# tjhladish/AbcSmc

Measured on AMD Instinct MI355X. Metric: particles/sec per SMC generation (PLS+weight+resample), 1/2/4/8 GPU, higher is better.
Workload: dtype f64 (inputs, model, distances, proposals, results; pair sums of the weight stage: fp64 operands as three f16 limbs on the matrix pipe + f32 v_exp_f32, weights <= 5e-7 rel of the fp64 oracle, largest seen 3.1e-7); 1 GPU; configs[2]: synthetic 1M particles x 16 params x 32 metrics, PLS 8 components, full generation; particles_per_gpu=1000000, particles_total=1000000, metrics=32, params=16, pls_components=8, pred_prior_size=100000, prev_pred_prior_size=100000, next_set_size=1000000, noise=MULTIVARIATE, ncomp_chosen=8, pls_component_rule=wilcoxon, parallelism=row-sharded x1, launcher=single GPU

## Files before the change

abcsmc_amd/csrc/select.hip:

```cpp
#include "abc_internal.h"

namespace {

struct SelState {
    unsigned long long prefix;
    unsigned long long mask;
    unsigned long long krem;
    unsigned long long n_less;
    unsigned long long ties;
};

__device__ __forceinline__ unsigned long long key_of(double d) {
    const unsigned long long b = (unsigned long long)__double_as_longlong(d);
    return (b >> 63) ? ~b : (b | 0x8000000000000000ull);
}
__device__ __forceinline__ double dist_of(unsigned long long k) {
    const unsigned long long b = (k >> 63) ? (k & 0x7fffffffffffffffull) : ~k;
    return __longlong_as_double((long long)b);
}

constexpr int SEL_BITS = 11;
constexpr int SEL_BINS = 1 << SEL_BITS;

__global__ void k_sel_init(SelState* st, unsigned long long K, unsigned int* hist) {
    for (int i = threadIdx.x; i < SEL_BINS; i += blockDim.x) hist[i] = 0;
    if (threadIdx.x == 0) { st->prefix = 0; st->mask = 0; st->krem = K; st->n_less = 0; st->ties = 0; }
}

__global__ __launch_bounds__(256) void k_sel_hist(const double* __restrict__ dist, size_t n,
                                                  const SelState* __restrict__ st, int shift, int nbits,
                                                  unsigned int* __restrict__ hist) {
    __shared__ unsigned int lh[SEL_BINS];
    for (int i = threadIdx.x; i < SEL_BINS; i += 256) lh[i] = 0;
    __syncthreads();
    const unsigned long long prefix = st->prefix, mask = st->mask;
    const unsigned int dm = (1u << nbits) - 1u;
    const size_t stride = (size_t)gridDim.x * 256;
    const int lane = threadIdx.x & 63;
    const unsigned long long lt_mask = (lane == 0) ? 0ull : (~0ull >> (64 - lane));
    const size_t nround = (n + stride - 1) / stride;
    for (size_t it = 0; it < nround; it++) {
        const size_t i = it * stride + (size_t)blockIdx.x * 256 + threadIdx.x;
        const unsigned long long k = (i < n) ? key_of(dist[i]) : 0ull;
        const bool in = (i < n) && ((k & mask) == prefix);
        const unsigned int d = (unsigned int)(k >> shift) & dm;
        unsigned long long peers = __ballot(in);
        for (int b = 0; b < nbits; b++) {
            const unsigned long long m = __ballot((d >> b) & 1u);
            peers &= ((d >> b) & 1u) ? m : ~m;
        }
        if (in && (peers & lt_mask) == 0) atomicAdd(&lh[d], (unsigned int)__popcll(peers));
    }
    __syncthreads();
    for (int i = threadIdx.x; i < SEL_BINS; i += 256) {
        const unsigned int c = lh[i];
        if (c) atomicAdd(&hist[i], c);
    }
}

__device__ __forceinline__ SelState sel_pick_block(const unsigned int* __restrict__ hist, SelState st, int shift, int nbits,
                                                   int last, unsigned long long K, unsigned long long* csum ,
                                                   int* found_digit, unsigned long long* found_below) {
    const int t = threadIdx.x;
    const int bins = 1 << nbits;
    const int per = (bins + 255) / 256;
    unsigned long long loc = 0;
    for (int j = 0; j < per; j++) { const int b = t * per + j; if (b < bins) loc += hist[b]; }
    const int lane = t & 63, wave = t >> 6;
    unsigned long long inc = loc;
#pragma unroll
    for (int o = 1; o < 64; o <<= 1) {
        const unsigned long long up = __shfl_up(inc, o, 64);
        if (lane >= o) inc += up;
    }
    if (lane == 63) csum[wave] = inc;
    __syncthreads();
    unsigned long long run = inc - loc;
    for (int w = 0; w < wave; w++) run += csum[w];
    const unsigned long long krem = st.krem;
    for (int j = 0; j < per; j++) {
        const int b = t * per + j;
        if (b < bins) {
            const unsigned long long c = hist[b];
            if (run < krem && krem <= run + c) { *found_digit = b; *found_below = run; }
            run += c;
        }
    }
    __syncthreads();
    const unsigned long long dm = ((1ull << nbits) - 1ull) << shift;
    st.prefix |= ((unsigned long long)*found_digit) << shift;
    st.mask |= dm;
    st.krem = krem - *found_below;
    if (last) { st.ties = st.krem; st.n_less = K - st.krem; }
    __syncthreads();
    return st;
}

__global__ __launch_bounds__(256) void k_sel_pick(SelState* st, int shift, int nbits, unsigned int* hist,
                                                  int last, unsigned long long K) {
    __shared__ unsigned long long csum[256];
    __shared__ int found_digit;
    __shared__ unsigned long long found_below;
    const SelState nst = sel_pick_block(hist, *st, shift, nbits, last, K, csum, &found_digit, &found_below);
    if (threadIdx.x == 0) *st = nst;
    for (int i = threadIdx.x; i < SEL_BINS; i += 256) hist[i] = 0;
}

__global__ void k_sel_init_fused(SelState* st_arr , unsigned long long K, unsigned int* hist_all ) {
    for (int i = threadIdx.x; i < 6 * SEL_BINS; i += blockDim.x) hist_all[i] = 0;
    if (threadIdx.x == 0) { st_arr[0].prefix = 0; st_arr[0].mask = 0; st_arr[0].krem = K; st_arr[0].n_less = 0; st_arr[0].ties = 0; }
}

__global__ __launch_bounds__(256) void k_sel_hist_fused(const double* __restrict__ dist, size_t n, SelState* __restrict__ st_arr,
                                                        int p, int shift_prev, int nbits_prev, int shift, int nbits,
                                                        unsigned int* __restrict__ hist_all, unsigned long long K) {
    __shared__ unsigned int lh[SEL_BINS];
    __shared__ unsigned long long csum[256];
    __shared__ int found_digit;
    __shared__ unsigned long long found_below;
    SelState st = st_arr[p > 0 ? p - 1 : 0];
    if (p > 0) {
        st = sel_pick_block(hist_all + (size_t)(p - 1) * SEL_BINS, st, shift_prev, nbits_prev, 0, K, csum, &found_digit, &found_below);
        if (threadIdx.x == 0) st_arr[p] = st;
    }
    for (int i = threadIdx.x; i < SEL_BINS; i += 256) lh[i] = 0;
    __syncthreads();
    unsigned int* hist = hist_all + (size_t)p * SEL_BINS;
    const unsigned long long prefix = st.prefix, mask = st.mask;
    const unsigned int dm = (1u << nbits) - 1u;
    const size_t stride = (size_t)gridDim.x * 256;
    const int lane = threadIdx.x & 63;
    const unsigned long long lt_mask = (lane == 0) ? 0ull : (~0ull >> (64 - lane));
    const size_t nround = (n + stride - 1) / stride;
    for (size_t it = 0; it < nround; it++) {
        const size_t i = it * stride + (size_t)blockIdx.x * 256 + threadIdx.x;
        const unsigned long long k = (i < n) ? key_of(dist[i]) : 0ull;
        const bool in = (i < n) && ((k & mask) == prefix);
        const unsigned int d = (unsigned int)(k >> shift) & dm;
        unsigned long long peers = __ballot(in);
        for (int b = 0; b < nbits; b++) {
            const unsigned long long m = __ballot((d >> b) & 1u);
            peers &= ((d >> b) & 1u) ? m : ~m;
        }
        if (in && (peers & lt_mask) == 0) atomicAdd(&lh[d], (unsigned int)__popcll(peers));
    }
    __syncthreads();
    for (int i = threadIdx.x; i < SEL_BINS; i += 256) {
        const unsigned int c = lh[i];
        if (c) atomicAdd(&hist[i], c);
    }
}


constexpr int BS_NB = 4096;
constexpr int BS_NB_BIG = 16384;
constexpr int BS_S = 4096;
constexpr int BS_CAP = 1024;
constexpr int BS_CSTRIDE = 32;
struct BinSel {
    unsigned long long lo, hi;
    int shift;
    int bstar;
    unsigned long long need;
    int fail;
    int pad_;
};

__global__ __launch_bounds__(1024) void k_bs_sample(const double* __restrict__ dist, size_t n, unsigned long long K,
                                                    BinSel* __restrict__ bs, unsigned int* __restrict__ hist ,
                                                    int* __restrict__ fail_flag, int nbins) {
    __shared__ unsigned long long sk[BS_S];
    __shared__ unsigned int h[256];
    __shared__ unsigned long long red[16];
    __shared__ unsigned long long s_prefix;
    __shared__ unsigned int s_rank;
    const int t = threadIdx.x;
    for (int i = t; i < nbins + 1; i += 1024) hist[i] = 0;
    const size_t stride = n / BS_S;
    unsigned long long mn = ~0ull;
    {
        static_assert(BS_S % 1024 == 0 && BS_S / 1024 <= 8, "samples per thread");
        double dv[BS_S / 1024];
#pragma unroll
        for (int j = 0; j < BS_S / 1024; j++) dv[j] = dist[(size_t)(t + 1024 * j) * stride + stride / 2];
#pragma unroll
        for (int j = 0; j < BS_S / 1024; j++) {
            const unsigned long long k = key_of(dv[j]);
            sk[t + 1024 * j] = k;
            mn = k < mn ? k : mn;
        }
    }
#pragma unroll
    for (int o = 32; o >= 1; o >>= 1) { const unsigned long long v = __shfl_xor(mn, o, 64); mn = v < mn ? v : mn; }
    if ((t & 63) == 0) red[t >> 6] = mn;
    const double f = (double)K / (double)n;
    double qd = f * BS_S + 4.0 * sqrt(BS_S * f * (1.0 - f)) + 8.0;
    unsigned int q = (qd >= (double)(BS_S - 1)) ? BS_S - 1 : (unsigned int)qd;
    if (t == 0) { s_prefix = 0; s_rank = q; }
    __syncthreads();
    for (int w = 0; w < 16; w++) mn = red[w] < mn ? red[w] : mn;
    unsigned long long mask = 0;
    for (int pass = 0; pass < 3; pass++) {
        const int shift = 56 - 8 * pass;
        if (t < 256) h[t] = 0;
        __syncthreads();
        const unsigned long long prefix = s_prefix;
        for (int i = t; i < BS_S; i += 1024)
            if ((sk[i] & mask) == prefix) atomicAdd(&h[(unsigned int)(sk[i] >> shift) & 255u], 1u);
        __syncthreads();
        if (t < 64) {
            unsigned int c[4], sum = 0;
#pragma unroll
            for (int j = 0; j < 4; j++) { c[j] = h[4 * t + j]; sum += c[j]; }
            unsigned int inc = sum;
#pragma unroll
            for (int o = 1; o < 64; o <<= 1) { const unsigned int u = __shfl_up(inc, o, 64); if (t >= o) inc += u; }
            unsigned int run = inc - sum;
            const unsigned int r = s_rank;
#pragma unroll
            for (int j = 0; j < 4; j++) {
                if (run <= r && r < run + c[j]) { s_prefix = prefix | ((unsigned long long)(4 * t + j) << shift); s_rank = r - run; }
                run += c[j];
            }
        }
        mask |= 255ull << shift;
        __syncthreads();
    }
    if (t == 0) {
        const unsigned long long lo = mn, hi = s_prefix | ~mask;
        const unsigned long long span = hi - lo;
        int shift = 0;
        while (shift < 63 && (span >> shift) >= (unsigned long long)(nbins - 1)) shift++;
        bs->lo = lo; bs->hi = hi; bs->shift = shift; bs->bstar = 0; bs->need = 0; bs->fail = 0; bs->pad_ = 0;
        *fail_flag = 0;
    }
}

__device__ __forceinline__ int bs_bin(unsigned long long k, unsigned long long lo, int shift) {
    return (k <= lo) ? 0 : (int)((k - lo) >> shift);
}

__global__ __launch_bounds__(256) void k_bs_hist(const double* __restrict__ dist, size_t n, const BinSel* __restrict__ bs,
                                                 unsigned int* __restrict__ hist, unsigned int* __restrict__ cursor, int nbins) {
    extern __shared__ unsigned int lh[];
    for (size_t i = (size_t)blockIdx.x * 256 + threadIdx.x; i < (size_t)nbins * BS_CSTRIDE; i += (size_t)gridDim.x * 256) cursor[i] = 0;
    for (int i = threadIdx.x; i < nbins; i += 256) lh[i] = 0;
    __syncthreads();
    const unsigned long long lo = bs->lo, hi = bs->hi;
    const int shift = bs->shift;
    const size_t stride = (size_t)gridDim.x * 256;
    for (size_t i0 = (size_t)blockIdx.x * 256 + threadIdx.x; i0 < n; i0 += 8 * stride) {
        double d[8];
#pragma unroll
        for (int u = 0; u < 8; u++) { const size_t i = i0 + u * stride; d[u] = dist[i < n ? i : i0]; }
#pragma unroll
        for (int u = 0; u < 8; u++) {
            const unsigned long long k = key_of(d[u]);
            if (i0 + u * stride < n && k <= hi) atomicAdd(&lh[bs_bin(k, lo, shift)], 1u);
        }
    }
    __syncthreads();
    for (int i = threadIdx.x; i < nbins; i += 256) {
        const unsigned int c = lh[i];
        if (c) atomicAdd(&hist[i], c);
    }
}

template <int BPT>
__global__ __launch_bounds__(1024) void k_bs_scan(BinSel* __restrict__ bs, unsigned int* __restrict__ hist, unsigned long long K,
                                                  int* __restrict__ fail_flag) {
    __shared__ unsigned int wsum[16];
    __shared__ int s_fail;
    const int t = threadIdx.x, lane = t & 63, wave = t >> 6;
    if (t == 0) s_fail = 0;
    unsigned int c[BPT], sum = 0;
#pragma unroll
    for (int j = 0; j < BPT; j++) { c[j] = hist[BPT * t + j]; sum += c[j]; }
    unsigned int inc = sum;
#pragma unroll
    for (int o = 1; o < 64; o <<= 1) { const unsigned int u = __shfl_up(inc, o, 64); if (lane >= o) inc += u; }
    if (lane == 63) wsum[wave] = inc;
    __syncthreads();
    unsigned int run = inc - sum;
    for (int w = 0; w < wave; w++) run += wsum[w];
    unsigned int tot = 0;
    for (int w = 0; w < 16; w++) tot += wsum[w];
#pragma unroll
    for (int j = 0; j < BPT; j++) {
        const unsigned int off = run;
        hist[BPT * t + j] = off;
        if ((unsigned long long)off < K && K <= (unsigned long long)off + c[j]) { bs->bstar = BPT * t + j; bs->need = K - off; }
        if ((unsigned long long)off < K && c[j] > (unsigned int)BS_CAP) s_fail = 1;
        run += c[j];
    }
    if (t == 0) hist[BPT * 1024] = tot;
    __syncthreads();
    if (t == 0) {
        const int fail = (s_fail || (unsigned long long)tot < K) ? 1 : 0;
        bs->fail = fail;
        *fail_flag = fail;
    }
}

__global__ __launch_bounds__(256) void k_bs_scatter(const double* __restrict__ dist, size_t n, const BinSel* __restrict__ bs,
                                                    const unsigned int* __restrict__ offs, unsigned int* __restrict__ cursor,
                                                    unsigned long long idx_base, unsigned long long* __restrict__ tkey,
                                                    unsigned long long* __restrict__ tidx) {
    if (bs->fail) return;
    const unsigned long long lo = bs->lo, hi = bs->hi;
    const int shift = bs->shift, bstar = bs->bstar;
    const size_t i = (size_t)blockIdx.x * 256 + threadIdx.x;
    if (i >= n) return;
    const unsigned long long k = key_of(dist[i]);
    if (k > hi) return;
    const int b = bs_bin(k, lo, shift);
    if (b > bstar) return;
    const unsigned int p = offs[b] + atomicAdd(&cursor[(size_t)b * BS_CSTRIDE], 1u);
    tkey[p] = k;
    tidx[p] = idx_base + i;
}

__global__ __launch_bounds__(256) void k_bs_sort(const BinSel* __restrict__ bs, const unsigned int* __restrict__ offs,
                                                 const unsigned long long* __restrict__ tkey,
                                                 const unsigned long long* __restrict__ tidx, unsigned long long K,
                                                 unsigned long long idx_base, unsigned long long* __restrict__ oidx,
                                                 double* __restrict__ odist) {
    __shared__ unsigned long long sk[BS_CAP];
    __shared__ unsigned long long si[BS_CAP];
    const int b = blockIdx.x, t = threadIdx.x;
    if (bs->fail) {
        for (unsigned long long i = (unsigned long long)b * 256 + t; i < K; i += (unsigned long long)gridDim.x * 256) {
            oidx[i] = idx_base + i;
            if (odist) odist[i] = 0.0;
        }
        return;
    }
    if (b > bs->bstar) return;
    const unsigned int o0 = offs[b], cnt = offs[b + 1] - o0;
    if (cnt == 0) return;
    const unsigned int keep = (b == bs->bstar) ? (unsigned int)bs->need : cnt;
    unsigned int n2 = 2;
    while (n2 < cnt) n2 <<= 1;
    for (unsigned int e = t; e < n2; e += 256) {
        sk[e] = (e < cnt) ? tkey[o0 + e] : ~0ull;
        si[e] = (e < cnt) ? tidx[o0 + e] : ~0ull;
    }
    __syncthreads();
    for (unsigned int k = 2; k <= n2; k <<= 1)
        for (unsigned int j = k >> 1; j > 0; j >>= 1) {
            for (unsigned int p = t; p < n2 / 2; p += 256) {
                const unsigned int i = ((p & ~(j - 1)) << 1) | (p & (j - 1));
                const unsigned long long ka = sk[i], kb = sk[i + j], ia = si[i], ib = si[i + j];
                const bool gt = (ka > kb) || (ka == kb && ia > ib);
                if (gt == ((i & k) == 0)) { sk[i] = kb; sk[i + j] = ka; si[i] = ib; si[i + j] = ia; }
            }
            __syncthreads();
        }
    for (unsigned int e = t; e < keep; e += 256) {
        oidx[o0 + e] = si[e];
        if (odist) odist[o0 + e] = dist_of(sk[e]);
    }
}

constexpr int CP_ITEMS = 8;
constexpr int CP_CHUNK = 256 * CP_ITEMS;

__global__ __launch_bounds__(256) void k_cp_count(const double* __restrict__ dist, size_t n,
                                                  SelState* __restrict__ st,
                                                  unsigned int* __restrict__ cnt , int nb,
                                                  const unsigned int* __restrict__ last_hist = nullptr, int shift = 0,
                                                  int nbits = 0, unsigned long long K = 0) {
    __shared__ unsigned int sl[4], se[4];
    __shared__ unsigned long long csum[256];
    __shared__ int found_digit;
    __shared__ unsigned long long found_below;
    unsigned long long T;
    if (last_hist) {
        const SelState fin = sel_pick_block(last_hist, st[0], shift, nbits, 1, K, csum, &found_digit, &found_below);
        if (threadIdx.x == 0) st[1] = fin;
        T = fin.prefix;
    } else {
        T = st->prefix;
    }
    const size_t base = (size_t)blockIdx.x * CP_CHUNK + (size_t)threadIdx.x * CP_ITEMS;
    unsigned int l = 0, e = 0;
#pragma unroll
    for (int j = 0; j < CP_ITEMS; j++) {
        const size_t i = base + j;
        if (i < n) { const unsigned long long k = key_of(dist[i]); l += (k < T); e += (k == T); }
    }
#pragma unroll
    for (int o = 32; o >= 1; o >>= 1) { l += __shfl_xor(l, o, 64); e += __shfl_xor(e, o, 64); }
    if ((threadIdx.x & 63) == 0) { sl[threadIdx.x >> 6] = l; se[threadIdx.x >> 6] = e; }
    __syncthreads();
    if (threadIdx.x == 0) {
        cnt[blockIdx.x] = sl[0] + sl[1] + sl[2] + sl[3];
        cnt[nb + blockIdx.x] = se[0] + se[1] + se[2] + se[3];
    }
}

__global__ __launch_bounds__(256) void k_scan_u32(unsigned int* __restrict__ a, int m0, int m1,
                                                  unsigned long long* __restrict__ totals = nullptr) {
    __shared__ unsigned int s[256];
    __shared__ unsigned int carry;
    for (int seg = 0; seg < 2; seg++) {
        unsigned int* p = seg ? a + m0 : a;
        const int m = seg ? m1 : m0;
        if (threadIdx.x == 0) carry = 0;
        __syncthreads();
        for (int b0 = 0; b0 < m; b0 += 256) {
            const int i = b0 + threadIdx.x;
            const unsigned int v = (i < m) ? p[i] : 0u;
            s[threadIdx.x] = v;
            __syncthreads();
            for (int o = 1; o < 256; o <<= 1) {
                const unsigned int add = (threadIdx.x >= o) ? s[threadIdx.x - o] : 0u;
                __syncthreads();
                s[threadIdx.x] += add;
                __syncthreads();
            }
            const unsigned int incl = s[threadIdx.x];
            const unsigned int c = carry;
            if (i < m) p[i] = c + incl - v;
            __syncthreads();
            if (threadIdx.x == 255) carry = c + incl;
            __syncthreads();
        }
        if (totals && threadIdx.x == 0) totals[seg] = carry;
        __syncthreads();
    }
}

__global__ __launch_bounds__(256) void k_cp_write(const double* __restrict__ dist, size_t n,
                                                  const SelState* __restrict__ st,
                                                  const unsigned int* __restrict__ off ,
                                                  int nb, unsigned long long idx_base,
                                                  unsigned long long* __restrict__ okey,
                                                  unsigned long long* __restrict__ oidx,
                                                  const unsigned long long* __restrict__ lim = nullptr,
                                                  unsigned long long cap = ~0ull ) {
    __shared__ unsigned int wl[4], we[4];
    const unsigned long long T = st->prefix, n_less = lim ? lim[0] : st->n_less, ties = lim ? lim[1] : st->ties;
    const int t = threadIdx.x, lane = t & 63, wave = t >> 6;
    const size_t base = (size_t)blockIdx.x * CP_CHUNK + (size_t)t * CP_ITEMS;
    unsigned long long k[CP_ITEMS];
    unsigned int l = 0, e = 0;
#pragma unroll
    for (int j = 0; j < CP_ITEMS; j++) {
        const size_t i = base + j;
        k[j] = (i < n) ? key_of(dist[i]) : ~0ull;
        if (i < n) { l += (k[j] < T); e += (k[j] == T); }
    }
    unsigned int il = l, ie = e;
#pragma unroll
    for (int o = 1; o < 64; o <<= 1) {
        const unsigned int al = __shfl_up(il, o, 64), ae = __shfl_up(ie, o, 64);
        if (lane >= o) { il += al; ie += ae; }
    }
    if (lane == 63) { wl[wave] = il; we[wave] = ie; }
    __syncthreads();
    unsigned int pl = il - l, pe = ie - e;
    for (int w = 0; w < wave; w++) { pl += wl[w]; pe += we[w]; }
    unsigned long long posl = (unsigned long long)off[blockIdx.x] + pl;
    unsigned long long pose = (unsigned long long)off[nb + blockIdx.x] + pe;
#pragma unroll
    for (int j = 0; j < CP_ITEMS; j++) {
        const size_t i = base + j;
        if (i >= n) break;
        if (k[j] < T) { if (posl < cap) { okey[posl] = k[j]; oidx[posl] = idx_base + i; } posl++; }
        else if (k[j] == T) {
            if (pose < ties) { okey[n_less + pose] = k[j]; oidx[n_less + pose] = idx_base + i; }
            pose++;
        }
    }
}

__global__ __launch_bounds__(256) void k_init_pairs(const double* __restrict__ dist, size_t n,
                                                    unsigned long long idx_base,
                                                    unsigned long long* __restrict__ okey,
                                                    unsigned long long* __restrict__ oidx) {
    const size_t i = (size_t)blockIdx.x * 256 + threadIdx.x;
    if (i < n) { okey[i] = key_of(dist[i]); if (oidx) oidx[i] = idx_base + i; }
}

__global__ __launch_bounds__(256) void k_keys_to_dist(const unsigned long long* __restrict__ key, size_t n,
                                                      double* __restrict__ dist) {
    const size_t i = (size_t)blockIdx.x * 256 + threadIdx.x;
    if (i < n) dist[i] = dist_of(key[i]);
}

constexpr int ST_ITEMS = 8;
constexpr int ST_CHUNK = 256 * ST_ITEMS;

__global__ __launch_bounds__(256) void k_sort_hist(const unsigned long long* __restrict__ key, size_t n, int shift,
                                                   unsigned int* __restrict__ bh , int nb) {
    __shared__ unsigned int lh[256];
    lh[threadIdx.x] = 0;
    __syncthreads();
    const size_t base = (size_t)blockIdx.x * ST_CHUNK;
#pragma unroll
    for (int j = 0; j < ST_ITEMS; j++) {
        const size_t i = base + (size_t)j * 256 + threadIdx.x;
        if (i < n) atomicAdd(&lh[(unsigned int)(key[i] >> shift) & 255u], 1u);
    }
    __syncthreads();
    bh[(size_t)threadIdx.x * nb + blockIdx.x] = lh[threadIdx.x];
}

__global__ __launch_bounds__(256) void k_sort_scatter(const unsigned long long* __restrict__ key,
                                                      const unsigned long long* __restrict__ idx, size_t n,
                                                      int shift, const unsigned int* __restrict__ bh, int nb,
                                                      const unsigned int* __restrict__ dtot,
                                                      unsigned long long* __restrict__ okey,
                                                      unsigned long long* __restrict__ oidx) {
    __shared__ unsigned int whist[4][256];
    __shared__ volatile unsigned int woff[4][256];
    __shared__ unsigned int dsum[4];
    const int t = threadIdx.x, lane = t & 63, wave = t >> 6;
#pragma unroll
    for (int w = 0; w < 4; w++) whist[w][t] = 0;
    const unsigned int mytot = dtot[t];
    unsigned int dinc = mytot;
#pragma unroll
    for (int o = 1; o < 64; o <<= 1) { const unsigned int a = __shfl_up(dinc, o, 64); if (lane >= o) dinc += a; }
    if (lane == 63) dsum[wave] = dinc;
    __syncthreads();
    unsigned int dbase = dinc - mytot;
#pragma unroll
    for (int w = 0; w < 4; w++) if (w < wave) dbase += dsum[w];
    const size_t seg = (size_t)blockIdx.x * ST_CHUNK + (size_t)wave * (ST_CHUNK / 4);
    unsigned long long k[ST_ITEMS];
#pragma unroll
    for (int j = 0; j < ST_ITEMS; j++) {
        const size_t i = seg + (size_t)j * 64 + lane;
        k[j] = (i < n) ? key[i] : 0ull;
        if (i < n) atomicAdd(&whist[wave][(unsigned int)(k[j] >> shift) & 255u], 1u);
    }
    __syncthreads();
    {
        unsigned int run = dbase + bh[(size_t)t * nb + blockIdx.x];
#pragma unroll
        for (int w = 0; w < 4; w++) { woff[w][t] = run; run += whist[w][t]; }
    }
    __syncthreads();
    const unsigned long long lt_mask = (lane == 0) ? 0ull : (~0ull >> (64 - lane));
#pragma unroll
    for (int j = 0; j < ST_ITEMS; j++) {
        const size_t i = seg + (size_t)j * 64 + lane;
        const bool valid = i < n;
        const unsigned int d = (unsigned int)(k[j] >> shift) & 255u;
        unsigned long long peers = __ballot(valid);
#pragma unroll
        for (int b = 0; b < 8; b++) {
            const unsigned long long m = __ballot((d >> b) & 1u);
            peers &= ((d >> b) & 1u) ? m : ~m;
        }
        if (valid) {
            const unsigned int rank = __popcll(peers & lt_mask);
            const unsigned int pos = woff[wave][d] + rank;
            okey[pos] = k[j];
            oidx[pos] = idx[i];
        }
        __builtin_amdgcn_wave_barrier();
        if (valid && (peers & lt_mask) == 0) woff[wave][d] += (unsigned int)__popcll(peers);
        __builtin_amdgcn_wave_barrier();
    }
}

__global__ __launch_bounds__(256) void k_sort_scan(unsigned int* __restrict__ bh, int nb, unsigned int* __restrict__ dtot) {
    __shared__ unsigned int wsum[4];
    const int d = blockIdx.x, t = threadIdx.x;
    unsigned int* row = bh + (size_t)d * nb;
    const int per = (nb + 255) / 256, i0 = t * per;
    unsigned int loc = 0;
    for (int c = 0; c < per; c++) if (i0 + c < nb) loc += row[i0 + c];
    unsigned int inc = loc;
#pragma unroll
    for (int o = 1; o < 64; o <<= 1) { const unsigned int a = __shfl_up(inc, o, 64); if ((t & 63) >= o) inc += a; }
    if ((t & 63) == 63) wsum[t >> 6] = inc;
    __syncthreads();
    unsigned int run = inc - loc;
#pragma unroll
    for (int w = 0; w < 4; w++) if (w < (t >> 6)) run += wsum[w];
    for (int c = 0; c < per; c++)
        if (i0 + c < nb) { const unsigned int v = row[i0 + c]; row[i0 + c] = run; run += v; }
    if (t == 255) dtot[d] = run;
}

constexpr int SC_N = 4096;
constexpr size_t SC_MAX_N = (size_t)1 << 18;

__global__ __launch_bounds__(1024) void k_sort_chunks(const unsigned long long* key, const unsigned long long* idx, size_t n,
                                                      unsigned long long* okey, unsigned long long* oidx) {
    __shared__ unsigned long long sk[SC_N];
    __shared__ unsigned long long si[SC_N];
    const size_t base = (size_t)blockIdx.x * SC_N;
    const unsigned cnt = (unsigned)((n - base < (size_t)SC_N) ? n - base : (size_t)SC_N);
    for (unsigned e = threadIdx.x; e < SC_N; e += 1024) {
        sk[e] = (e < cnt) ? key[base + e] : ~0ull;
        si[e] = ((e < cnt) ? idx[base + e] : 0ull) | ((unsigned long long)e << 48);
    }
    __syncthreads();
    unsigned prev_j = 1;
    for (unsigned k = 2; k <= SC_N; k <<= 1) {
        for (unsigned j = k >> 1; j > 0; j >>= 1) {
            if (j >= 128 || prev_j >= 128) __syncthreads(); else __builtin_amdgcn_wave_barrier();
            prev_j = j;
            unsigned ii[2];
            unsigned long long ka[2], kb[2], ia[2], ib[2];
#pragma unroll
            for (int m = 0; m < 2; m++) {
                const unsigned p = threadIdx.x + 1024u * m;
                ii[m] = ((p & ~(j - 1)) << 1) | (p & (j - 1));
                ka[m] = sk[ii[m]]; kb[m] = sk[ii[m] + j]; ia[m] = si[ii[m]]; ib[m] = si[ii[m] + j];
            }
#pragma unroll
            for (int m = 0; m < 2; m++) {
                const bool gt = (ka[m] > kb[m]) || (ka[m] == kb[m] && (ia[m] >> 48) > (ib[m] >> 48));
                if (gt == ((ii[m] & k) == 0)) { sk[ii[m]] = kb[m]; sk[ii[m] + j] = ka[m]; si[ii[m]] = ib[m]; si[ii[m] + j] = ia[m]; }
            }
        }
    }
    __syncthreads();
    for (unsigned e = threadIdx.x; e < cnt; e += 1024) {
        okey[base + e] = sk[e];
        oidx[base + e] = si[e] & 0x0000ffffffffffffull;
    }
}

__global__ __launch_bounds__(256) void k_merge_chunks(const unsigned long long* __restrict__ key,
                                                      const unsigned long long* __restrict__ idx, size_t n,
                                                      unsigned long long* __restrict__ okey, unsigned long long* __restrict__ oidx) {
    const size_t t = (size_t)blockIdx.x * 256 + threadIdx.x;
    if (t >= n) return;
    const unsigned q = (unsigned)(t / SC_N), W = (unsigned)((n + SC_N - 1) / SC_N);
    const unsigned long long x = key[t];
    size_t pos = t - (size_t)q * SC_N;
    for (unsigned r0 = 0; r0 < W; r0 += 8) {
        unsigned lo[8], len[8];
#pragma unroll
        for (int u = 0; u < 8; u++) {
            const unsigned r = r0 + u;
            lo[u] = 0;
            len[u] = (r < W && r != q) ? (unsigned)((n - (size_t)r * SC_N < (size_t)SC_N) ? n - (size_t)r * SC_N : (size_t)SC_N) : 0u;
        }
#pragma unroll 1
        for (unsigned step = SC_N; step >= 1; step >>= 1) {
            unsigned long long y[8];
#pragma unroll
            for (int u = 0; u < 8; u++) {
                const unsigned c = lo[u] + step;
                const unsigned r = (r0 + u < W) ? r0 + u : q;
                y[u] = key[(size_t)r * SC_N + ((c <= len[u]) ? c - 1 : 0u)];
            }
#pragma unroll
            for (int u = 0; u < 8; u++) {
                const unsigned c = lo[u] + step;
                const bool before = (r0 + u < q) ? (y[u] <= x) : (y[u] < x);
                lo[u] = (c <= len[u] && before) ? c : lo[u];
            }
        }
#pragma unroll
        for (int u = 0; u < 8; u++) pos += lo[u];
    }
    okey[pos] = x;
    oidx[pos] = idx[t];
}

int sort_pairs_u64(abc_ctx* ctx, unsigned long long* key0, unsigned long long* idx0, unsigned long long* key1,
                   unsigned long long* idx1, size_t n, int byte_lo = 0, int byte_hi = 8) {
    if (n <= 1) return ABC_OK;
    StageTimer tm(ctx, ST_SORT);
    if (byte_lo == 0 && byte_hi == 8 && n <= SC_MAX_N) {
        const unsigned nc = (unsigned)((n + SC_N - 1) / SC_N);
        if (nc == 1) {
            hipLaunchKernelGGL(k_sort_chunks, dim3(1), dim3(1024), 0, ctx->stream, key0, idx0, n, key0, idx0);
        } else {
            hipLaunchKernelGGL(k_sort_chunks, dim3(nc), dim3(1024), 0, ctx->stream, key0, idx0, n, key1, idx1);
            hipLaunchKernelGGL(k_merge_chunks, dim3((unsigned)((n + 255) / 256)), dim3(256), 0, ctx->stream, key1, idx1, n,
                               key0, idx0);
        }
        ABC_HIP(ctx, hipGetLastError());
        return ABC_OK;
    }
    const int nb = (int)((n + ST_CHUNK - 1) / ST_CHUNK);
    unsigned int* bh = (unsigned int*)abc_ws_alloc(ctx, ((size_t)256 * nb + 256) * sizeof(unsigned int));
    if (!bh) ABC_FAIL(ctx, ABC_ERR_NOMEM, "sort: workspace exhausted");
    unsigned int* dtot = bh + (size_t)256 * nb;
    unsigned long long *ka = key0, *ia = idx0, *kb = key1, *ib = idx1;
    for (int pass = byte_lo; pass < byte_hi; pass++) {
        const int shift = 8 * pass;
        hipLaunchKernelGGL(k_sort_hist, dim3(nb), dim3(256), 0, ctx->stream, ka, n, shift, bh, nb);
        hipLaunchKernelGGL(k_sort_scan, dim3(256), dim3(256), 0, ctx->stream, bh, nb, dtot);
        hipLaunchKernelGGL(k_sort_scatter, dim3(nb), dim3(256), 0, ctx->stream, ka, ia, n, shift, bh, nb, (const unsigned int*)dtot, kb, ib);
        unsigned long long* tk = ka; ka = kb; kb = tk;
        unsigned long long* ti = ia; ia = ib; ib = ti;
    }
    ABC_HIP(ctx, hipGetLastError());
    return ABC_OK;
}

}

int abc_sort_u64_bytes(abc_ctx* ctx, unsigned long long* key0, unsigned long long* val0, unsigned long long* key1,
                       unsigned long long* val1, size_t n, int byte_lo, int byte_hi) {
    if ((byte_hi - byte_lo) % 2 != 0) ABC_FAIL(ctx, ABC_ERR_INVALID, "sort: odd number of radix passes");
    return sort_pairs_u64(ctx, key0, val0, key1, val1, n, byte_lo, byte_hi);
}

static const int kSelShift[6] = {53, 42, 31, 20, 9, 0};
static const int kSelWidth[6] = {11, 11, 11, 11, 11, 9};

int launch_select_begin(abc_ctx* ctx, uint64_t K, long long* state, int* hist) {
    hipLaunchKernelGGL(k_sel_init, dim3(1), dim3(256), 0, ctx->stream, (SelState*)state, (unsigned long long)K,
                       (unsigned int*)hist);
    ABC_HIP(ctx, hipGetLastError());
    return ABC_OK;
}
int launch_select_hist(abc_ctx* ctx, const double* dist, size_t n, const long long* state, int pass, int* hist) {
    if (pass < 0 || pass > 5) ABC_FAIL(ctx, ABC_ERR_INVALID, "select: pass %d", pass);
    if (n == 0) return ABC_OK;
    StageTimer tm(ctx, ST_SELECT);
    size_t hb = (n + 255) / 256;
    if (hb > 512) hb = 512;
    hipLaunchKernelGGL(k_sel_hist, dim3((unsigned)hb), dim3(256), 0, ctx->stream, dist, n, (const SelState*)state,
                       kSelShift[pass], kSelWidth[pass], (unsigned int*)hist);
    ABC_HIP(ctx, hipGetLastError());
    return ABC_OK;
}
int launch_select_pick(abc_ctx* ctx, long long* state, int pass, int* hist, uint64_t K) {
    if (pass < 0 || pass > 5) ABC_FAIL(ctx, ABC_ERR_INVALID, "select: pass %d", pass);
    StageTimer tm(ctx, ST_SELECT);
    hipLaunchKernelGGL(k_sel_pick, dim3(1), dim3(256), 0, ctx->stream, (SelState*)state, kSelShift[pass], kSelWidth[pass],
                       (unsigned int*)hist, (int)(pass == 5), (unsigned long long)K);
    ABC_HIP(ctx, hipGetLastError());
    return ABC_OK;
}
int launch_select_count(abc_ctx* ctx, const double* dist, size_t n, const long long* state, long long* counts) {
    StageTimer tm(ctx, ST_SELECT);
    const int nb = (int)((n + CP_CHUNK - 1) / CP_CHUNK);
    unsigned int* cnt = (unsigned int*)abc_ws_alloc(ctx, (size_t)2 * (nb + 1) * sizeof(unsigned int));
    if (!cnt) ABC_FAIL(ctx, ABC_ERR_NOMEM, "select: workspace exhausted");
    if (nb) hipLaunchKernelGGL(k_cp_count, dim3(nb), dim3(256), 0, ctx->stream, dist, n, (SelState*)state, cnt, nb);
    hipLaunchKernelGGL(k_scan_u32, dim3(1), dim3(256), 0, ctx->stream, cnt, nb, nb, (unsigned long long*)counts);
    ABC_HIP(ctx, hipGetLastError());
    return ABC_OK;
}
int launch_select_compact(abc_ctx* ctx, const double* dist, size_t n, const long long* state, uint64_t n_less,
                          uint64_t ties_take, uint64_t idx_base, uint64_t* idx_out, double* dist_out) {
    StageTimer tm(ctx, ST_SELECT);
    const size_t nw = n_less + ties_take;
    if (nw == 0 || n == 0) return ABC_OK;
    const int nb = (int)((n + CP_CHUNK - 1) / CP_CHUNK);
    unsigned int* cnt = (unsigned int*)abc_ws_alloc(ctx, (size_t)2 * nb * sizeof(unsigned int));
    unsigned long long* lim = (unsigned long long*)abc_ws_alloc(ctx, 2 * sizeof(unsigned long long));
    unsigned long long* key = (unsigned long long*)abc_ws_alloc(ctx, nw * 8);
    if (!cnt || !lim || !key) ABC_FAIL(ctx, ABC_ERR_NOMEM, "select: workspace exhausted");
    const unsigned long long hl[2] = {n_less, ties_take};
    ABC_HIP(ctx, hipMemcpyAsync(lim, hl, sizeof(hl), hipMemcpyHostToDevice, ctx->stream));
    hipLaunchKernelGGL(k_cp_count, dim3(nb), dim3(256), 0, ctx->stream, dist, n, (SelState*)state, cnt, nb);
    hipLaunchKernelGGL(k_scan_u32, dim3(1), dim3(256), 0, ctx->stream, cnt, nb, nb, (unsigned long long*)nullptr);
    hipLaunchKernelGGL(k_cp_write, dim3(nb), dim3(256), 0, ctx->stream, dist, n, (const SelState*)state, cnt, nb,
                       (unsigned long long)idx_base, key, (unsigned long long*)idx_out, lim);
    hipLaunchKernelGGL(k_keys_to_dist, dim3((unsigned)((nw + 255) / 256)), dim3(256), 0, ctx->stream, key, nw, dist_out);
    ABC_HIP(ctx, hipGetLastError());
    return ABC_OK;
}

static int select_by_bins(abc_ctx* ctx, const double* dist, size_t n, size_t K, uint64_t idx_base, uint64_t* idx, double* dist_out) {
    if (!ctx->sel_fail_dev) ABC_HIP(ctx, hipMalloc((void**)&ctx->sel_fail_dev, sizeof(int)));
    int* const fail_dev = ctx->sel_fail_dev;
    const int nbins = K <= ((size_t)1 << 18) ? BS_NB : BS_NB_BIG;
    BinSel* bs = (BinSel*)abc_ws_alloc(ctx, sizeof(BinSel));
    unsigned int* hist = (unsigned int*)abc_ws_alloc(ctx, ((size_t)nbins + 1) * sizeof(unsigned int));
    unsigned int* cursor = (unsigned int*)abc_ws_alloc(ctx, (size_t)nbins * BS_CSTRIDE * sizeof(unsigned int));
    unsigned long long* tkey = (unsigned long long*)abc_ws_alloc(ctx, (K + BS_CAP) * 8);
    unsigned long long* tidx = (unsigned long long*)abc_ws_alloc(ctx, (K + BS_CAP) * 8);
    if (!bs || !hist || !cursor || !tkey || !tidx) ABC_FAIL(ctx, ABC_ERR_NOMEM, "select: workspace exhausted");
    StageTimer tm(ctx, ST_SELECT);
    hipLaunchKernelGGL(k_bs_sample, dim3(1), dim3(1024), 0, ctx->stream, dist, n, (unsigned long long)K, bs, hist, fail_dev, nbins);
    size_t hb = (n + 255) / 256;
    if (hb > 512) hb = 512;
    const size_t hl = (size_t)nbins * sizeof(unsigned int);
    if (hl > (48u << 10)) ABC_HIP(ctx, hipFuncSetAttribute((const void*)k_bs_hist, hipFuncAttributeMaxDynamicSharedMemorySize, (int)hl));
    hipLaunchKernelGGL(k_bs_hist, dim3((unsigned)hb), dim3(256), hl, ctx->stream, dist, n, (const BinSel*)bs, hist, cursor, nbins);
    if (nbins == BS_NB) hipLaunchKernelGGL(k_bs_scan<BS_NB / 1024>, dim3(1), dim3(1024), 0, ctx->stream, bs, hist, (unsigned long long)K, fail_dev);
    else hipLaunchKernelGGL(k_bs_scan<BS_NB_BIG / 1024>, dim3(1), dim3(1024), 0, ctx->stream, bs, hist, (unsigned long long)K, fail_dev);
    hipLaunchKernelGGL(k_bs_scatter, dim3((unsigned)((n + 255) / 256)), dim3(256), 0, ctx->stream, dist, n, (const BinSel*)bs,
                       (const unsigned int*)hist, cursor, (unsigned long long)idx_base, tkey, tidx);
    hipLaunchKernelGGL(k_bs_sort, dim3((unsigned)nbins), dim3(256), 0, ctx->stream, (const BinSel*)bs, (const unsigned int*)hist,
                       (const unsigned long long*)tkey, (const unsigned long long*)tidx, (unsigned long long)K,
                       (unsigned long long)idx_base, (unsigned long long*)idx, dist_out);
    ABC_HIP(ctx, hipGetLastError());
    return ABC_OK;
}

static int select_by_radix(abc_ctx* ctx, const double* dist, size_t n, size_t K, uint64_t idx_base, uint64_t* idx, double* dist_out) {
    unsigned long long* key0 = (unsigned long long*)abc_ws_alloc(ctx, K * 8);
    unsigned long long* key1 = (unsigned long long*)abc_ws_alloc(ctx, K * 8);
    unsigned long long* idx1 = (unsigned long long*)abc_ws_alloc(ctx, K * 8);
    if (!key0 || !key1 || !idx1) ABC_FAIL(ctx, ABC_ERR_NOMEM, "select: workspace exhausted");
    unsigned long long* idx0 = (unsigned long long*)idx;
    {
    StageTimer tm(ctx, ST_SELECT);
    if (K == n) {
        hipLaunchKernelGGL(k_init_pairs, dim3((unsigned)((n + 255) / 256)), dim3(256), 0, ctx->stream, dist, n,
                           (unsigned long long)idx_base, key0, idx0);
    } else {
        SelState* st = (SelState*)abc_ws_alloc(ctx, 7 * sizeof(SelState));
        unsigned int* hist = (unsigned int*)abc_ws_alloc(ctx, 6 * SEL_BINS * sizeof(unsigned int));
        const int nb = (int)((n + CP_CHUNK - 1) / CP_CHUNK);
        unsigned int* cnt = (unsigned int*)abc_ws_alloc(ctx, (size_t)2 * nb * sizeof(unsigned int));
        if (!st || !hist || !cnt) ABC_FAIL(ctx, ABC_ERR_NOMEM, "select: workspace exhausted");
        hipLaunchKernelGGL(k_sel_init_fused, dim3(1), dim3(256), 0, ctx->stream, st, (unsigned long long)K, hist);
        size_t hb = (n + 255) / 256;
        if (hb > 512) hb = 512;
        static const int shifts[6] = {53, 42, 31, 20, 9, 0};
        static const int widths[6] = {11, 11, 11, 11, 11, 9};
        for (int p = 0; p < 6; p++)
            hipLaunchKernelGGL(k_sel_hist_fused, dim3((unsigned)hb), dim3(256), 0, ctx->stream, dist, n, st, p,
                               p ? shifts[p - 1] : 0, p ? widths[p - 1] : 0, shifts[p], widths[p], hist, (unsigned long long)K);
        hipLaunchKernelGGL(k_cp_count, dim3(nb), dim3(256), 0, ctx->stream, dist, n, st + 5, cnt, nb,
                           (const unsigned int*)(hist + 5 * SEL_BINS), shifts[5], widths[5], (unsigned long long)K);
        hipLaunchKernelGGL(k_scan_u32, dim3(1), dim3(256), 0, ctx->stream, cnt, nb, nb, (unsigned long long*)nullptr);
        hipLaunchKernelGGL(k_cp_write, dim3(nb), dim3(256), 0, ctx->stream, dist, n, (const SelState*)(st + 6), cnt, nb,
                           (unsigned long long)idx_base, key0, idx0, (const unsigned long long*)nullptr);
    }
    }
    ABC_HIP(ctx, hipGetLastError());
    ABC_TRY(sort_pairs_u64(ctx, key0, idx0, key1, idx1, K));
    if (dist_out) {
        hipLaunchKernelGGL(k_keys_to_dist, dim3((unsigned)((K + 255) / 256)), dim3(256), 0, ctx->stream, key0, K,
                           dist_out);
        ABC_HIP(ctx, hipGetLastError());
    }
    return ABC_OK;
}

int launch_select_smallest(abc_ctx* ctx, const double* dist, size_t n, size_t K, uint64_t idx_base, uint64_t* idx,
                           double* dist_out, bool defer_check) {
    if (K == 0) return ABC_OK;
    if (K > n) ABC_FAIL(ctx, ABC_ERR_INVALID, "select: K = %zu > n = %zu", K, n);
    const bool bins = !ctx->sel_force_radix && n >= 4 * (size_t)BS_S && 2 * K <= n && K <= ((size_t)1 << 20);
    ctx->sel_bins_ran = bins;
    if (!bins) return select_by_radix(ctx, dist, n, K, idx_base, idx, dist_out);
    const size_t mark = ctx->ws_off;
    ctx->sel_bin_selections++;
    ABC_TRY(select_by_bins(ctx, dist, n, K, idx_base, idx, dist_out));
    if (defer_check) return ABC_OK;
    int failed = 0;
    ABC_TRY(abc_select_check(ctx, &failed));
    if (!failed) return ABC_OK;
    ctx->sel_bin_giveups++;
    ctx->ws_off = mark;
    return select_by_radix(ctx, dist, n, K, idx_base, idx, dist_out);
}

int abc_select_check_queue(abc_ctx* ctx, int* slot) {
    *slot = 0;
    if (!ctx->sel_bins_ran || !ctx->sel_fail_dev) return ABC_OK;
    ABC_HIP(ctx, hipMemcpyAsync(slot, ctx->sel_fail_dev, sizeof(int), hipMemcpyDeviceToHost, ctx->stream));
    return ABC_OK;
}
int abc_select_check_done(abc_ctx* ctx, const int* slot) {
    const int f = (ctx->sel_bins_ran && ctx->sel_fail_dev) ? *slot : 0;
    ctx->sel_bins_ran = false;
    return f;
}

int abc_select_check(abc_ctx* ctx, int* failed) {
    *failed = 0;
    if (!ctx->sel_bins_ran || !ctx->sel_fail_dev) return ABC_OK;
    int f = 0;
    ABC_HIP(ctx, hipMemcpyAsync(&f, ctx->sel_fail_dev, sizeof(int), hipMemcpyDeviceToHost, ctx->stream));
    ABC_HIP(ctx, hipStreamSynchronize(ctx->stream));
    ctx->sel_bins_ran = false;
    *failed = f;
    return ABC_OK;
}

__global__ __launch_bounds__(256) void k_merge_runs(const double* __restrict__ key, const unsigned long long* __restrict__ idx,
                                                    int W, size_t len, double* __restrict__ okey,
                                                    unsigned long long* __restrict__ oidx,
                                                    unsigned long long* __restrict__ osrc ) {
    const size_t t = (size_t)blockIdx.x * 256 + threadIdx.x;
    if (t >= (size_t)W * len) return;
    const int q = (int)(t / len);
    const size_t i = t - (size_t)q * len;
    const double d = key[t];
    const unsigned long long x = key_of(d);
    size_t top = 1;
    while (top < len) top <<= 1;
    size_t pos = i;
    for (int r0 = 0; r0 < W; r0 += 8) {
        size_t lo[8];
#pragma unroll
        for (int u = 0; u < 8; u++) lo[u] = 0;
#pragma unroll 1
        for (size_t step = top; step >= 1; step >>= 1) {
            unsigned long long y[8];
#pragma unroll
            for (int u = 0; u < 8; u++) {
                const int r = (r0 + u < W) ? r0 + u : q;
                const size_t c = lo[u] + step;
                y[u] = key_of(key[(size_t)r * len + ((c <= len) ? c - 1 : 0)]);
            }
#pragma unroll
            for (int u = 0; u < 8; u++) {
                const int r = r0 + u;
                const size_t c = lo[u] + step;
                const bool before = (r < q) ? (y[u] <= x) : (y[u] < x);
                lo[u] = (r < W && r != q && c <= len && before) ? c : lo[u];
            }
        }
#pragma unroll
        for (int u = 0; u < 8; u++) pos += lo[u];
    }
    okey[pos] = d;
    oidx[pos] = idx[t];
    if (osrc) osrc[pos] = t;
}

int launch_merge_runs(abc_ctx* ctx, const double* key, const uint64_t* idx, int W, size_t len, double* okey, uint64_t* oidx,
                      uint64_t* osrc) {
    if (W < 1) ABC_FAIL(ctx, ABC_ERR_INVALID, "merge: W = %d", W);
    const size_t n = (size_t)W * len;
    if (n == 0) return ABC_OK;
    StageTimer tm(ctx, ST_SORT);
    hipLaunchKernelGGL(k_merge_runs, dim3((unsigned)((n + 255) / 256)), dim3(256), 0, ctx->stream, key,
                       (const unsigned long long*)idx, W, len, okey, (unsigned long long*)oidx, (unsigned long long*)osrc);
    ABC_HIP(ctx, hipGetLastError());
    return ABC_OK;
}

int launch_sort_pairs(abc_ctx* ctx, double* key, uint64_t* idx, size_t n) {
    if (n <= 1) return ABC_OK;
    unsigned long long* key0 = (unsigned long long*)abc_ws_alloc(ctx, n * 8);
    unsigned long long* key1 = (unsigned long long*)abc_ws_alloc(ctx, n * 8);
    unsigned long long* idx1 = (unsigned long long*)abc_ws_alloc(ctx, n * 8);
    if (!key0 || !key1 || !idx1) ABC_FAIL(ctx, ABC_ERR_NOMEM, "sort: workspace exhausted");
    hipLaunchKernelGGL(k_init_pairs, dim3((unsigned)((n + 255) / 256)), dim3(256), 0, ctx->stream, key, n, 0ull, key0,
                       (unsigned long long*)nullptr);
    ABC_TRY(sort_pairs_u64(ctx, key0, (unsigned long long*)idx, key1, idx1, n));
    hipLaunchKernelGGL(k_keys_to_dist, dim3((unsigned)((n + 255) / 256)), dim3(256), 0, ctx->stream, key0, n, key);
    ABC_HIP(ctx, hipGetLastError());
    return ABC_OK;
}
```

Before: 365.6 million particles/s.

## Rank-sort small selection bins and streamline sample-quantile kernel with wave intrinsics

The per-bin sort in the bin-select path now uses rank counting for small bins instead of a full bitonic sort. Bins of up to 64 entries rank within one wave via readlane, and bins of up to 512 entries rank against LDS pairs using a carry-chain asm compare. The sample kernel keeps its samples in registers, uses wave-aggregated LDS atomics and DPP scans in place of the thread-0 shared handoffs and extra barriers, and computes the bin shift from leading-zero counts. Optional timestamp instrumentation is added behind a compile flag. The select stage is a small part of the whole generation, so the overall effect may be small, and the O(n^2) ranking could be slow for bins that are nearly full.

```diff
diff --git a/abcsmc_amd/csrc/select.hip b/abcsmc_amd/csrc/select.hip
--- a/abcsmc_amd/csrc/select.hip
+++ b/abcsmc_amd/csrc/select.hip
@@ -166,74 +166,136 @@
     int pad_;
 };
 
+#ifdef SEL_STAMPS
+constexpr int SEL_STAMP_WORDS = 16 + 8 * 16384;
+__device__ unsigned long long g_sel_stamps[SEL_STAMP_WORDS];
+#define SEL_STAMP_BEGIN(base) unsigned long long* const st_out_ = g_sel_stamps + (base); \
+        const unsigned long long st_t0_ = wall_clock64(); long long st_last_ = __builtin_readcyclecounter()
+#define SEL_STAMP(id) do { const long long now_ = __builtin_readcyclecounter(); \
+        if (threadIdx.x == 0) st_out_[id] = (unsigned long long)(now_ - st_last_); st_last_ = now_; } while (0)
+#define SEL_STAMP_WAIT() __builtin_amdgcn_s_waitcnt(0)
+#define SEL_STAMP_END(id0, id1) do { if (threadIdx.x == 0) { st_out_[id0] = st_t0_; st_out_[id1] = wall_clock64(); } } while (0)
+#define SEL_STAMP_SET(id, v) do { if (threadIdx.x == 0) st_out_[id] = (v); } while (0)
+#else
+#define SEL_STAMP_BEGIN(base)
+#define SEL_STAMP(id)
+#define SEL_STAMP_WAIT()
+#define SEL_STAMP_END(id0, id1)
+#define SEL_STAMP_SET(id, v)
+#endif
+
+__device__ __forceinline__ unsigned int bs_wave_scan(unsigned int v, int lane) {
+    v += (unsigned int)__builtin_amdgcn_update_dpp(0, (int)v, 0x111, 0xf, 0xf, true);
+    v += (unsigned int)__builtin_amdgcn_update_dpp(0, (int)v, 0x112, 0xf, 0xf, true);
+    v += (unsigned int)__builtin_amdgcn_update_dpp(0, (int)v, 0x114, 0xf, 0xf, true);
+    v += (unsigned int)__builtin_amdgcn_update_dpp(0, (int)v, 0x118, 0xf, 0xf, true);
+    const unsigned int r0 = (unsigned int)__builtin_amdgcn_readlane((int)v, 15), r1 = (unsigned int)__builtin_amdgcn_readlane((int)v, 31),
+                       r2 = (unsigned int)__builtin_amdgcn_readlane((int)v, 47);
+    const int row = lane >> 4;
+    return v + (row > 0 ? r0 : 0u) + (row > 1 ? r1 : 0u) + (row > 2 ? r2 : 0u);
+}
+
 __global__ __launch_bounds__(1024) void k_bs_sample(const double* __restrict__ dist, size_t n, unsigned long long K,
                                                     BinSel* __restrict__ bs, unsigned int* __restrict__ hist ,
                                                     int* __restrict__ fail_flag, int nbins) {
-    __shared__ unsigned long long sk[BS_S];
-    __shared__ unsigned int h[256];
+    __shared__ unsigned int h[3][256];
     __shared__ unsigned long long red[16];
-    __shared__ unsigned long long s_prefix;
-    __shared__ unsigned int s_rank;
-    const int t = threadIdx.x;
-    for (int i = t; i < nbins + 1; i += 1024) hist[i] = 0;
+    const int t = threadIdx.x, lane = t & 63;
+    SEL_STAMP_BEGIN(0);
     const size_t stride = n / BS_S;
     unsigned long long mn = ~0ull;
-    {
-        static_assert(BS_S % 1024 == 0 && BS_S / 1024 <= 8, "samples per thread");
-        double dv[BS_S / 1024];
-#pragma unroll
-        for (int j = 0; j < BS_S / 1024; j++) dv[j] = dist[(size_t)(t + 1024 * j) * stride + stride / 2];
-#pragma unroll
-        for (int j = 0; j < BS_S / 1024; j++) {
-            const unsigned long long k = key_of(dv[j]);
-            sk[t + 1024 * j] = k;
-            mn = k < mn ? k : mn;
-        }
-    }
-#pragma unroll
-    for (int o = 32; o >= 1; o >>= 1) { const unsigned long long v = __shfl_xor(mn, o, 64); mn = v < mn ? v : mn; }
-    if ((t & 63) == 0) red[t >> 6] = mn;
+    unsigned long long sk[BS_S / 1024];
+    static_assert(BS_S % 1024 == 0 && BS_S / 1024 <= 8, "samples per thread");
+    double dv[BS_S / 1024];
+#pragma unroll
+    for (int j = 0; j < BS_S / 1024; j++) dv[j] = dist[(size_t)(t + 1024 * j) * stride + stride / 2];
+    for (int i = t; i < nbins + 1; i += 1024) hist[i] = 0;
+    if (t < 3 * 256) (&h[0][0])[t] = 0;
     const double f = (double)K / (double)n;
     double qd = f * BS_S + 4.0 * sqrt(BS_S * f * (1.0 - f)) + 8.0;
     unsigned int q = (qd >= (double)(BS_S - 1)) ? BS_S - 1 : (unsigned int)qd;
-    if (t == 0) { s_prefix = 0; s_rank = q; }
-    __syncthreads();
-    for (int w = 0; w < 16; w++) mn = red[w] < mn ? red[w] : mn;
-    unsigned long long mask = 0;
+#pragma unroll
+    for (int j = 0; j < BS_S / 1024; j++) {
+        const unsigned long long k = key_of(dv[j]);
+        sk[j] = k;
+        mn = k < mn ? k : mn;
+    }
+#pragma unroll
+    for (int o = 32; o >= 1; o >>= 1) { const unsigned long long v = __shfl_xor(mn, o, 64); mn = v < mn ? v : mn; }
+    if (lane == 0) red[t >> 6] = mn;
+    SEL_STAMP(0);
+    __syncthreads();
+    SEL_STAMP(1);
+    unsigned long long mask = 0, s_prefix = 0;
+    unsigned int s_rank = q;
     for (int pass = 0; pass < 3; pass++) {
         const int shift = 56 - 8 * pass;
-        if (t < 256) h[t] = 0;
+        const unsigned long long prefix = s_prefix;
+        bool in[BS_S / 1024], same = true;
+        unsigned int d[BS_S / 1024];
+#pragma unroll
+        for (int j = 0; j < BS_S / 1024; j++) {
+            in[j] = (sk[j] & mask) == prefix;
+            d[j] = (unsigned int)(sk[j] >> shift) & 255u;
+        }
+        const unsigned int d_first = (unsigned int)__builtin_amdgcn_readfirstlane((int)d[0]);
+#pragma unroll
+        for (int j = 0; j < BS_S / 1024; j++) same = same && in[j] && d[j] == d_first;
+        if (__ballot(!same) == 0) {
+            if (lane == 0) atomicAdd(&h[pass][d_first], 64u * (BS_S / 1024));
+        } else {
+#pragma unroll
+            for (int j = 0; j < BS_S / 1024; j++) {
+                const unsigned long long act = __ballot(in[j]);
+                if (act == 0) continue;
+                const int first = __ffsll((long long)act) - 1;
+                const unsigned int d0 = (unsigned int)__builtin_amdgcn_readlane((int)d[j], first);
+                const unsigned long long peers = __ballot(in[j] && d[j] == d0);
+                if (lane == first) atomicAdd(&h[pass][d0], (unsigned int)__popcll(peers));
+                else if (in[j] && d[j] != d0) atomicAdd(&h[pass][d[j]], 1u);
+            }
+        }
         __syncthreads();
-        const unsigned long long prefix = s_prefix;
-        for (int i = t; i < BS_S; i += 1024)
-            if ((sk[i] & mask) == prefix) atomicAdd(&h[(unsigned int)(sk[i] >> shift) & 255u], 1u);
-        __syncthreads();
-        if (t < 64) {
+        SEL_STAMP(3 + 3 * pass);
+        {
             unsigned int c[4], sum = 0;
 #pragma unroll
-            for (int j = 0; j < 4; j++) { c[j] = h[4 * t + j]; sum += c[j]; }
-            unsigned int inc = sum;
-#pragma unroll
-            for (int o = 1; o < 64; o <<= 1) { const unsigned int u = __shfl_up(inc, o, 64); if (t >= o) inc += u; }
-            unsigned int run = inc - sum;
+            for (int j = 0; j < 4; j++) { c[j] = h[pass][4 * lane + j]; sum += c[j]; }
+            unsigned int run = bs_wave_scan(sum, lane) - sum;
             const unsigned int r = s_rank;
+            unsigned int digit = 0, below = 0;
+            bool mine = false;
 #pragma unroll
             for (int j = 0; j < 4; j++) {
-                if (run <= r && r < run + c[j]) { s_prefix = prefix | ((unsigned long long)(4 * t + j) << shift); s_rank = r - run; }
+                if (run <= r && r < run + c[j]) { digit = 4 * lane + j; below = run; mine = true; }
                 run += c[j];
             }
+            const unsigned long long owner = __ballot(mine);
+            if (owner) {
+                const int src = __ffsll((long long)owner) - 1;
+                s_prefix = prefix | ((unsigned long long)(unsigned int)__builtin_amdgcn_readlane((int)digit, src) << shift);
+                s_rank = r - (unsigned int)__builtin_amdgcn_readlane((int)below, src);
+            }
         }
         mask |= 255ull << shift;
-        __syncthreads();
+        SEL_STAMP(4 + 3 * pass);
+    }
+    if (t < 64) {
+        mn = red[lane & 15];
+#pragma unroll
+        for (int o = 8; o >= 1; o >>= 1) { const unsigned long long v = __shfl_xor(mn, o, 64); mn = v < mn ? v : mn; }
     }
     if (t == 0) {
         const unsigned long long lo = mn, hi = s_prefix | ~mask;
         const unsigned long long span = hi - lo;
-        int shift = 0;
+        const int bits_span = span ? 64 - __clzll((long long)span) : 0, bits_nb = 32 - __clz(nbins - 1);
+        int shift = bits_span > bits_nb ? bits_span - bits_nb : 0;
         while (shift < 63 && (span >> shift) >= (unsigned long long)(nbins - 1)) shift++;
         bs->lo = lo; bs->hi = hi; bs->shift = shift; bs->bstar = 0; bs->need = 0; bs->fail = 0; bs->pad_ = 0;
         *fail_flag = 0;
     }
+    SEL_STAMP(11);
+    SEL_STAMP_END(12, 13);
 }
 
 __device__ __forceinline__ int bs_bin(unsigned long long k, unsigned long long lo, int shift) {
@@ -320,25 +382,116 @@
     tidx[p] = idx_base + i;
 }
 
+constexpr int BS_RANK_WAVE = 64;
+constexpr int BS_RANK_WG = 512;
+static_assert(BS_RANK_WG == 2 * 256 && BS_RANK_WG <= BS_CAP, "at most two pairs per thread of k_bs_sort");
+
+__device__ __forceinline__ void bs_count_below(unsigned int& rank, unsigned long long kj, unsigned long long ij, unsigned long long k,
+                                               unsigned long long ix) {
+    unsigned int diff;
+    asm("v_sub_co_u32 %1, vcc, %2, %6\n\t"
+        "v_subb_co_u32 %1, vcc, %3, %7, vcc\n\t"
+        "v_subb_co_u32 %1, vcc, %4, %8, vcc\n\t"
+        "v_subb_co_u32 %1, vcc, %5, %9, vcc\n\t"
+        "v_addc_co_u32 %0, vcc, 0, %0, vcc"
+        : "+v"(rank), "=&v"(diff)
+        : "v"((unsigned int)ij), "v"((unsigned int)(ij >> 32)), "v"((unsigned int)kj), "v"((unsigned int)(kj >> 32)),
+          "v"((unsigned int)ix), "v"((unsigned int)(ix >> 32)), "v"((unsigned int)k), "v"((unsigned int)(k >> 32))
+        : "vcc");
+}
+
+template <int E>
+__device__ __forceinline__ void bs_rank_lds(const unsigned long long* sp, unsigned int cnt, const unsigned long long (&k)[2],
+                                            const unsigned long long (&ix)[2], unsigned int (&rank)[2]) {
+    const ulonglong2* const pairs = reinterpret_cast<const ulonglong2*>(sp);
+    unsigned int j = 0;
+    for (; j + 8 <= cnt; j += 8) {
+        ulonglong2 pj[8];
+#pragma unroll
+        for (int u = 0; u < 8; u++) pj[u] = pairs[j + u];
+#pragma unroll
+        for (int u = 0; u < 8; u++)
+#pragma unroll
+            for (int e = 0; e < E; e++) bs_count_below(rank[e], pj[u].x, pj[u].y, k[e], ix[e]);
+    }
+    for (; j < cnt; j++) {
+        const ulonglong2 pj = pairs[j];
+#pragma unroll
+        for (int e = 0; e < E; e++) bs_count_below(rank[e], pj.x, pj.y, k[e], ix[e]);
+    }
+}
+
+__device__ __forceinline__ unsigned long long bs_readlane(unsigned long long v, int j) {
+    const unsigned int lo = (unsigned int)__builtin_amdgcn_readlane((int)(unsigned int)v, j);
+    const unsigned int hi = (unsigned int)__builtin_amdgcn_readlane((int)(unsigned int)(v >> 32), j);
+    return ((unsigned long long)hi << 32) | lo;
+}
+
 __global__ __launch_bounds__(256) void k_bs_sort(const BinSel* __restrict__ bs, const unsigned int* __restrict__ offs,
                                                  const unsigned long long* __restrict__ tkey,
                                                  const unsigned long long* __restrict__ tidx, unsigned long long K,
                                                  unsigned long long idx_base, unsigned long long* __restrict__ oidx,
                                                  double* __restrict__ odist) {
-    __shared__ unsigned long long sk[BS_CAP];
-    __shared__ unsigned long long si[BS_CAP];
-    const int b = blockIdx.x, t = threadIdx.x;
+    __shared__ __align__(16) unsigned long long sp[2 * BS_CAP];
+    unsigned long long* const sk = sp;
+    unsigned long long* const si = sp + BS_CAP;
+    const int b = gridDim.x - 1 - blockIdx.x, t = threadIdx.x;
+    SEL_STAMP_BEGIN(16 + 8 * blockIdx.x);
     if (bs->fail) {
-        for (unsigned long long i = (unsigned long long)b * 256 + t; i < K; i += (unsigned long long)gridDim.x * 256) {
+        for (unsigned long long i = (unsigned long long)blockIdx.x * 256 + t; i < K; i += (unsigned long long)gridDim.x * 256) {
             oidx[i] = idx_base + i;
             if (odist) odist[i] = 0.0;
         }
         return;
     }
-    if (b > bs->bstar) return;
+    if (b > bs->bstar) { SEL_STAMP_END(5, 6); return; }
     const unsigned int o0 = offs[b], cnt = offs[b + 1] - o0;
-    if (cnt == 0) return;
+    SEL_STAMP(0);
+    SEL_STAMP_SET(7, 1ull + cnt);
+    if (cnt == 0) { SEL_STAMP_END(5, 6); return; }
     const unsigned int keep = (b == bs->bstar) ? (unsigned int)bs->need : cnt;
+    if (cnt <= (unsigned int)BS_RANK_WAVE) {
+        if (t >= 64) return;
+        const unsigned long long k = ((unsigned int)t < cnt) ? tkey[o0 + t] : ~0ull, ix = ((unsigned int)t < cnt) ? tidx[o0 + t] : ~0ull;
+        SEL_STAMP_WAIT();
+        SEL_STAMP(1);
+        unsigned int rank = 0;
+        for (unsigned int j = 0; j < cnt; j++) {
+            const unsigned long long kj = bs_readlane(k, (int)j), ij = bs_readlane(ix, (int)j);
+            rank += (unsigned int)((kj < k) | ((kj == k) & (ij < ix)));
+        }
+        SEL_STAMP(2);
+        if ((unsigned int)t < cnt && rank < keep) {
+            oidx[o0 + rank] = ix;
+            if (odist) odist[o0 + rank] = dist_of(k);
+        }
+        SEL_STAMP(3);
+        SEL_STAMP_END(5, 6);
+        return;
+    }
+    if (cnt <= (unsigned int)BS_RANK_WG) {
+        unsigned long long k[2] = {~0ull, ~0ull}, ix[2] = {~0ull, ~0ull};
+        unsigned int rank[2] = {0, 0};
+#pragma unroll
+        for (int e = 0; e < 2; e++) {
+            const unsigned int p = t + 256 * e;
+            if (p < cnt) { k[e] = tkey[o0 + p]; ix[e] = tidx[o0 + p]; sp[2 * p] = k[e]; sp[2 * p + 1] = ix[e]; }
+        }
+        __syncthreads();
+        SEL_STAMP(1);
+        if (cnt <= 256) bs_rank_lds<1>(sp, cnt, k, ix, rank);
+        else bs_rank_lds<2>(sp, cnt, k, ix, rank);
+#pragma unroll
+        for (int e = 0; e < 2; e++) {
+            if (t + 256 * e < cnt && rank[e] < keep) {
+                oidx[o0 + rank[e]] = ix[e];
+                if (odist) odist[o0 + rank[e]] = dist_of(k[e]);
+            }
+        }
+        SEL_STAMP(2);
+        SEL_STAMP_END(5, 6);
+        return;
+    }
     unsigned int n2 = 2;
     while (n2 < cnt) n2 <<= 1;
     for (unsigned int e = t; e < n2; e += 256) {
@@ -346,6 +499,7 @@
         si[e] = (e < cnt) ? tidx[o0 + e] : ~0ull;
     }
     __syncthreads();
+    SEL_STAMP(1);
     for (unsigned int k = 2; k <= n2; k <<= 1)
         for (unsigned int j = k >> 1; j > 0; j >>= 1) {
             for (unsigned int p = t; p < n2 / 2; p += 256) {
@@ -356,10 +510,13 @@
             }
             __syncthreads();
         }
+    SEL_STAMP(2);
     for (unsigned int e = t; e < keep; e += 256) {
         oidx[o0 + e] = si[e];
         if (odist) odist[o0 + e] = dist_of(sk[e]);
     }
+    SEL_STAMP(3);
+    SEL_STAMP_END(5, 6);
 }
 
 constexpr int CP_ITEMS = 8;
@@ -794,6 +951,16 @@
     ABC_HIP(ctx, hipGetLastError());
     return ABC_OK;
 }
+
+#ifdef SEL_STAMPS
+extern "C" int abc_debug_select_stamps(unsigned long long* out) {
+    if (hipDeviceSynchronize() != hipSuccess) return -1;
+    if (hipMemcpyFromSymbol(out, HIP_SYMBOL(g_sel_stamps), sizeof(unsigned long long) * SEL_STAMP_WORDS) != hipSuccess) return -1;
+    void* p = nullptr;
+    if (hipGetSymbolAddress(&p, HIP_SYMBOL(g_sel_stamps)) != hipSuccess) return -1;
+    return hipMemset(p, 0, sizeof(unsigned long long) * SEL_STAMP_WORDS) == hipSuccess ? 0 : -1;
+}
+#endif
 
 static int select_by_radix(abc_ctx* ctx, const double* dist, size_t n, size_t K, uint64_t idx_base, uint64_t* idx, double* dist_out) {
     unsigned long long* key0 = (unsigned long long*)abc_ws_alloc(ctx, K * 8);
```

Result: no change. 365.6 million particles/s (-0.0%).
